# YannisLamp/crypto-recommendation

Measured on AMD Instinct MI355X. Metric: point hash+assign ops/sec at d=128, N=10M, K=256; 1/2/4/8 MI355X, higher is better.
Workload: dtype fp32 points; split-f16 MFMA scores (f32 accumulate); tuples, bucket IDs and cluster IDs bit-exact (x87-exact hashing, certified argmin); distances: certified f32, <= 2^-20 relative to the reference's fp64 (north star: 1e-5; the context's default LSHKM_DIST_CERTIFIED mode), LSHKM_DIST_EXACT for the r; 1 GPU; C3 Lloyd K=256 + C2 LSH L=5 k=4 hashing, N=10000000 per GPU, d=128; N_per_gpu=10000000, N_total=10000000, d=128, K=256, L=5, k=4, nb=100000, parallelism=dp1 (row shards)

## Files before the change

### crypto-recommendation_amd/csrc/fused.hip

```cpp
#include "../../include/lshkm.h"
#include "fused_impl.h"
#include "index.h"

namespace lshkm {

namespace {

struct FusedPlan {
    bool hash = false, cos = false;
    int rows = 0;
    int nblk = 0;
    int64_t seg_rows = 0;
    int np_hi = 0;
    int np_refine = 0;
};

int fused_workspace(lshkm_ctx ctx, const FusedShape& sh, FusedWorkspace& w) {
    const FusedLayout l = fused_layout(sh);
    int rc;
    struct { Buf& b; size_t bytes; } const bufs[] = {
        {ctx->ws_c32, l.c16},      {ctx->ws_cconst, l.cconst}, {ctx->ws_ambig, l.list1}, {ctx->ws_counter, l.counter},
        {ctx->ws_seg, l.seg1},     {ctx->ws_hfix, l.fix},      {ctx->ws_seg3, l.seg3},   {ctx->ws_part, l.part},
        {ctx->ws_ambig2, l.list2}, {ctx->ws_seg2, l.seg2},     {ctx->ws_tuples, l.tuples}, {ctx->ws_cf32, l.cf32},
        {ctx->ws_c64p, l.c64p},    {ctx->ws_xn2, l.xn2}};
// ... 6 lines not shown
    w.nbv = (double*)at(ctx->ws_cconst, l.nbv_off);
    if (l.cf32) { w.C32 = (float*)at(ctx->ws_cf32, 0); w.rn32 = (float*)at(ctx->ws_cf32, l.rn32_off); }
    if (l.c64p) w.C64p = ctx->ws_c64p.as<double>();
    w.list1 = ctx->ws_ambig.as<int32_t>(); w.seg1 = ctx->ws_seg.as<int32_t>();
    w.list2 = ctx->ws_ambig2.as<int32_t>(); w.seg2 = ctx->ws_seg2.as<int32_t>();
    if (l.seg3) w.seg3 = ctx->ws_seg3.as<int32_t>();
    w.hfix = (unsigned long long*)at(ctx->ws_hfix, l.hfix_off);
    w.cfix = (unsigned long long*)at(ctx->ws_hfix, l.cfix_off);
    w.hfix2 = (unsigned long long*)at(ctx->ws_hfix, l.hfix2_off);
    if (l.part) w.part = ctx->ws_part.as<float4>();
    w.cnt = ctx->ws_counter.as<unsigned long long>();
    if (l.xn2) w.xn2 = ctx->ws_xn2.as<double>();
    if (l.tuples) w.tuples = ctx->ws_tuples.as<int32_t>();
    return 0;
}

FusedArgs fused_common_args(lshkm_ctx ctx, const AssignRequest& q, const FusedShape& sh, const FusedWorkspace& w) {
    FusedArgs a{};
    a.X = q.X.f64 ? nullptr : q.X.f(); a.X64 = q.X.f64 ? q.X.d() : nullptr;
    a.N = q.N; a.d = q.d;
    a.xvec = sh.rows == 1 ? (a.d % 4 == 0 && ((uintptr_t)a.X & 15) == 0) : (a.d % 2 == 0 && ((uintptr_t)a.X64 & 15) == 0);
    a.Ch = w.Ch; a.Cl = w.Cl; a.cnh = w.cnh; a.cbound = w.cbound; a.Kpad = sh.Kpad();
    a.C64 = w.C64p ? w.C64p : q.C; a.Cd = q.C;
    a.C32 = w.C32; a.rn32 = w.rn32; a.fast_dist = sh.fast ? 1 : 0;
    a.assign = q.assign; a.dist = q.dist;
    a.stats = ctx->stats.as<unsigned long long>();
    a.nb = 1;
    if (q.lsh) {
        const ProjTable& pj = q.lsh->proj;
        a.Vh = pj.vh_d.as<_Float16>(); a.Vl = pj.vl_d.as<_Float16>(); a.PT = pj.PT_d.as<double>();
        a.tv = pj.t_d.as<float>(); a.pnorm = pj.pn_d.as<double>(); a.v1 = pj.v1_d.as<double>();
        a.rv = pj.r_d.as<int32_t>(); a.w = pj.w; a.L = pj.L; a.k = pj.k; a.LK = pj.LK; a.LKpad = pj.LKpad;
        a.nb = q.lsh->nb;
    }
    a.bdiv = make_bucket_div(a.nb);
    if (sh.cosine) { a.nbv = w.nbv; a.xn2 = w.xn2; }
    a.cfix = w.cfix; a.cfix_counts = w.seg3; a.cfix_count = w.cfix ? w.cnt + CNT_CFIX : nullptr;
    a.pass_first = 1; a.pass_last = 1;
    return a;
}

void hash_outputs(FusedArgs& a, const AssignRequest& q, const FusedShape& sh, const FusedWorkspace& w) {
    a.hfix = w.hfix; a.hfix_count = w.hfix ? w.cnt + CNT_HFIX : nullptr;
    if (!q.lsh) return;
    a.phi = q.phi; a.bucket = q.bucket;
    a.tuples = sh.cosine ? nullptr : q.tuples ? q.tuples : w.tuples;
}

template <typename T>
DevList<T> segmented(T* p, unsigned long long* count, int32_t* counts, const AssignRequest& q, const FusedPlan& plan) {
    DevList<T> l;
    l.p = p; l.count = count; l.bound = q.N; l.counts = counts;
    l.seg_rows = plan.seg_rows; l.nseg = plan.nblk;
    return l;
}

int fused_hi_passes(hipStream_t s, const FusedArgs& hi, const FusedPlan& p) {
    const bool gather_on = !test_switch("LSHKM_GATHER", "0");
    int rc;
    if (p.rows != 0) {
        HiForm h;
        h.metric = p.cos; h.rows = p.rows;
        h.fast = !p.cos && hi.fast_dist;
        h.gath = !p.cos && !h.fast && p.rows == 1 && hi.Kpad <= FH_GATH_KMAX && gather_on;
        return launch_fused_hi_pass(s, p.nblk, h, hi);
    }
    if (!p.cos && p.np_hi == 2 && test_switch("LSHKM_HI_TWO_IMAGE", "1")) {
        HiForm h;
        h.hash = p.hash; h.two_image = true;
        return launch_fused_hi_pass(s, p.nblk, h, hi);
    }
    for (int i = 0; i < p.np_hi; i++) {
        const int c0 = i * FH_KMAX;
        FusedArgs a = hi;
        a.Ch = hi.Ch + (size_t)c0 * FU_D; a.cnh = hi.cnh + c0;
        a.Kpad = std::min(FH_KMAX, hi.Kpad - c0);
        a.t0 = c0 / 32; a.pass_first = i == 0; a.pass_last = i == p.np_hi - 1;
        HiForm h;
        h.hash = p.hash && i == 0; h.mp = p.np_hi > 1; h.metric = p.cos;
        if (!p.cos && !h.mp) {
            const bool small = a.Kpad <= FH_GATH_KMAX && gather_on;
            h.fast = small && a.fast_dist;
            h.gath = small && !a.fast_dist;
        } else if (!p.cos) {
            h.fast = !h.hash && a.fast_dist && a.pass_last;
        }
        if ((rc = launch_fused_hi_pass(s, p.nblk, h, a))) return rc;
    }
    return 0;
}

int fused_refine_passes(hipStream_t s, const FusedArgs& rf, const FusedPlan& p) {
    for (int i = 0; i < p.np_refine; i++) {
        const int c0 = i * FP_KMAX;
        FusedArgs r = rf;
        r.Ch = rf.Ch + (size_t)c0 * FU_D; r.Cl = rf.Cl + (size_t)c0 * FU_D; r.cnh = rf.cnh + c0;
        r.Kpad = std::min(FP_KMAX, rf.Kpad - c0);
        r.t0 = c0 / 32; r.pass_first = i == 0; r.pass_last = i == p.np_refine - 1;
        const int rc = launch_fused_refine_pass(s, (unsigned)p.nblk, p.cos, p.np_refine > 1, p.rows, r);
        if (rc) return rc;
    }
    return 0;
}

struct SideFork {
    lshkm_ctx c;
    bool open = false;
    int fork() {
        if (hipEventRecord(c->fork_ev, c->stream) != hipSuccess ||
            hipStreamWaitEvent(c->side_stream, c->fork_ev, 0) != hipSuccess)
            return kstatus("fused_assign (fork)");
        open = true;
        return 0;
    }
    int end_side() {
        if (c->timing) {
            if (hipEventRecord(c->tev[2], c->side_stream) != hipSuccess) return kstatus("fused_assign (timing)");
            c->tev_side = true;
        }
        if (hipEventRecord(c->join_ev, c->side_stream) != hipSuccess) return kstatus("fused_assign (join)");
        return 0;
    }
    int join() {
        if (!open) return 0;
        if (hipStreamWaitEvent(c->stream, c->join_ev, 0) != hipSuccess) return kstatus("fused_assign (join)");
        open = false;
        return 0;
    }
    ~SideFork() { if (open) (void)hipStreamSynchronize(c->side_stream); }
};

#ifdef LSHKM_PHASE_TIMING
struct PhaseReport {
    hipStream_t s;
    unsigned long long* d = nullptr;
    explicit PhaseReport(hipStream_t s_) : s(s_) {
        static unsigned long long* prof_d = nullptr;
        if (!prof_d) (void)hipMalloc(&prof_d, 64);
        (void)hipMemsetAsync(prof_d, 0, 64, s);
        d = prof_d;
    }
    ~PhaseReport() {
        unsigned long long v[6];
        (void)hipMemcpyAsync(v, d, 48, hipMemcpyDeviceToHost, s);
        (void)hipStreamSynchronize(s);
        fprintf(stderr, "PHASES %llu %llu %llu %llu %llu\n", v[0], v[1], v[2], v[3], v[4]);
    }
};
#endif

}

int fused_assign(lshkm_ctx ctx, const AssignRequest& q) {
    hipStream_t s = ctx->stream;
    const bool cosine = q.metric != LSHKM_METRIC_EUCLIDEAN;
    const ProjTable* pj = q.lsh ? &q.lsh->proj : nullptr;
    const FusedRoute route = fused_route(cosine, q.X.f64, q.d, q.K, pj != nullptr, pj ? pj->k : 0, pj ? pj->LK : 0,
                                         test_switch("LSHKM_FUSED_FORM", "chunked"));
    if (route.form == FusedForm::none || (pj && (q.lsh->metric != q.metric || !pj->mfma_ok))) {
        set_error("fused_assign: no fused form runs this shape (fused_route, fused_layout.h)");
        return LSHKM_ERR_ARG;
    }
    FusedShape sh;
    sh.N = q.N; sh.d = q.d; sh.K = q.K; sh.cosine = cosine; sh.rows = route.rows;
    sh.hash = pj != nullptr; sh.LK = pj ? pj->LK : 0;
    sh.fast = !cosine && sh.rows != 2 && !q.force_exact && ctx->dist_mode == LSHKM_DIST_CERTIFIED;
// ... 92 lines not shown
```

### crypto-recommendation_amd/csrc/fused_hi.hip

```cpp
#include "fused_impl.h"

namespace lshkm {

__host__ __device__ constexpr int fh_lds_bytes(int Kpad, bool hash) {
    return 16 + Kpad * FU_RS * 2 + Kpad * 4 + (hash ? 2 * 32 * FU_RS * 2 + FP_HC_BYTES : 0);
}
static_assert(fh_lds_bytes(FH_KMAX, true) <= 160 * 1024, "hi-only LDS image exceeds 160 KiB");
constexpr double FH_A = 130.0 * 0x1p-23;

constexpr int FH_WAVES_MPFAST = 12;
constexpr int FH_FAST_WAVES = 8;
template <bool HASH, bool MP, int MET, bool FAST = false>
__host__ __device__ constexpr int fh_waves() {
    return HASH && MP ? 12 : (MP && FAST ? FH_WAVES_MPFAST : (FAST && !MP ? FH_FAST_WAVES : 8));
}

__device__ inline int cosine_halves_finish(double sh0, double sl0, double ts0, double sh, double sl, double ts,
                                           double xa, double nbv, double& v) {
    const double mb = 2.0 * sqrt(__dmul_rn(xa, nbv)) * (1.0 + 0x1p-40);
    const double tsum = __dadd_rn(ts0, ts);
    if (!(tsum >= 0x1p-790)) return 2;
    IpAcc ip;
    const double t = __dadd_rn(sh0, sh);
    const double bb = __dsub_rn(t, sh0);
// ... 37 lines not shown
    for (int j = 0; j < 4; j++) cb[j] = *reinterpret_cast<const double2*>(crow_h + 2 * j);
#pragma unroll
    for (int s = 0; s < 8; s++) {
        double cv[8];
#pragma unroll
        for (int j = 0; j < 4; j++) { cv[2 * j] = cb[j].x; cv[2 * j + 1] = cb[j].y; }
        if (s + 1 < 8) {
#pragma unroll
            for (int j = 0; j < 4; j++) cb[j] = *reinterpret_cast<const double2*>(crow_h + 16 * (s + 1) + 2 * j);
        }
#pragma unroll
        for (int j = 0; j < 8; j++) {
            const double pj = __dmul_rn((double)xf[8 * s + j], cv[j]);
            const double t = __dadd_rn(sh, pj);
            const double bb = __dsub_rn(t, sh);
            const double e = __dadd_rn(__dsub_rn(sh, __dsub_rn(t, bb)), __dsub_rn(pj, bb));
            sh = t;
            sl = __dadd_rn(sl, e);
            ts = __dadd_rn(ts, fabs(__dadd_rn(t, off)));
        }
        const double other = swap_halves(sh, h);
        if (h == 1) ts = __dadd_rn(ts, 8.0 * fabs(__dsub_rn(other, off)));
        off = other;
    }
    const double sh0 = swap_halves(sh, h), sl0 = swap_halves(sl, h), ts0 = swap_halves(ts, h);
    if (h == 0) return 2;
    return cosine_halves_finish(sh0, sl0, ts0, sh, sl, ts, xa, nbv, v);
}

__device__ inline int cosine_winner_halves_x64(const FusedArgs& a, int64_t rowc, const double* __restrict__ crow_h,
                                               double nbv, int h, double& v) {
    double2 xn[4], xnn[4];
    load_x64_step(a, rowc, 0, h, xn);
    load_x64_step(a, rowc, 1, h, xnn);
    double sh = 0.0, sl = 0.0, ts = 0.0;
    double off = 0.0;
    double2 cb[4];
#pragma unroll
    for (int j = 0; j < 4; j++) cb[j] = *reinterpret_cast<const double2*>(crow_h + 2 * j);
#pragma unroll 1
    for (int s = 0; s < 8; s++) {
        double xv[8], cv[8];
#pragma unroll
        for (int j = 0; j < 4; j++) {
            xv[2 * j] = xn[j].x; xv[2 * j + 1] = xn[j].y;
            cv[2 * j] = cb[j].x; cv[2 * j + 1] = cb[j].y;
            xn[j] = xnn[j];
        }
        if (s + 2 < 8) load_x64_step(a, rowc, s + 2, h, xnn);
        if (s + 1 < 8) {
#pragma unroll
            for (int j = 0; j < 4; j++) cb[j] = *reinterpret_cast<const double2*>(crow_h + 16 * (s + 1) + 2 * j);
        }
#pragma unroll
        for (int j = 0; j < 8; j++) {
            const double pj = __dmul_rn(xv[j], cv[j]);
            const double t = __dadd_rn(sh, pj);
            const double bb = __dsub_rn(t, sh);
            const double e = __dadd_rn(__dsub_rn(sh, __dsub_rn(t, bb)), __dsub_rn(pj, bb));
            sh = t;
            sl = __dadd_rn(sl, e);
            ts = __dadd_rn(ts, fabs(__dadd_rn(t, off)));
        }
        const double other = swap_halves(sh, h);
        if (h == 1) ts = __dadd_rn(ts, 8.0 * fabs(__dsub_rn(other, off)));
        off = other;
    }
    const double sh0 = swap_halves(sh, h), sl0 = swap_halves(sl, h), ts0 = swap_halves(ts, h);
    if (h == 0) return 2;
    return cosine_halves_finish(sh0, sl0, ts0, sh, sl, ts, a.xn2[rowc], nbv, v);
}

constexpr int FH_GATH_STEP = 32 * 16 * 8;
constexpr int FH_GATH_WAVE = 2 * FH_GATH_STEP;
__host__ __device__ constexpr int fh_gath_off(int Kpad, bool hash) { return (fh_lds_bytes(Kpad, hash) + 255) & ~255; }
static_assert(fh_gath_off(FH_GATH_KMAX, true) + 8 * FH_GATH_WAVE <= 160 * 1024, "gather ring exceeds 160 KiB");

__device__ inline void glds16(const void* gsrc, uint32_t lds_dst) {
    unsigned keep;
    asm volatile("s_mov_b32 %0, m0\n\ts_mov_b32 m0, %2\n\ts_nop 0\n\tglobal_load_lds_dwordx4 %1, off\n\ts_mov_b32 m0, %0"
                 : "=&s"(keep) : "v"(gsrc), "s"(lds_dst) : "memory");
}

template <bool HASH, bool MP = false, int MET = 0, int NIMG = 1, bool GATH = false, int ROWS = 0, bool FAST = false>
__global__ __launch_bounds__((64 * fh_waves<HASH, MP, MET, FAST>()), 1) void fused_hi_kernel(FusedArgs a) {
    constexpr int FH_WAVES = fh_waves<HASH, MP, MET, FAST>();
    constexpr int FH_THREADS = 64 * FH_WAVES;
    static_assert(NIMG == 1 || (!MP && MET == 0), "two-image form: euclidean, single launch");
    static_assert(!GATH || (!MP && MET == 0 && NIMG == 1 && FH_WAVES == 8), "gather ring: euclidean single pass");
    static_assert(ROWS == 0 || (!HASH && !MP && NIMG == 1), "general rows: Lloyd without hashing, one pass");
    static_assert(!(GATH && ROWS == 2), "fp64 rows re-read x in the chain: register loads of the winner rows");
    static_assert(!FAST || (MET == 0 && ROWS != 2 && NIMG == 1 && !GATH), "fast distance: euclidean, fp32 rows");
    extern __shared__ __attribute__((aligned(16))) char smem[];
    const int Kpad = a.Kpad;
    const bool fastd = FAST || a.fast_dist != 0;
    const int KI = NIMG == 2 ? FH_KMAX : Kpad;
    int* lcount = reinterpret_cast<int*>(smem);
    _Float16* lch = reinterpret_cast<_Float16*>(smem + 16);
    float* lcn = reinterpret_cast<float*>(lch + KI * FU_RS);
    _Float16* lvh = reinterpret_cast<_Float16*>(lcn + KI);
    _Float16* lvl = lvh + 32 * FU_RS;
    float* lpn0 = reinterpret_cast<float*>(lvl + 32 * FU_RS);
    float* lv10 = lpn0 + 32;
    float* lt0 = lv10 + 32;
    int32_t* lr0 = reinterpret_cast<int32_t*>(lt0 + 32);

    auto load_image = [&](int img) {
        const int r0 = img * KI, nr = NIMG == 2 && img == 1 ? Kpad - FH_KMAX : KI;
        constexpr int FH_CU = 8;
        for (int e0 = 0; e0 < nr * 16; e0 += FH_THREADS * FH_CU) {
            float4 v[FH_CU];
#pragma unroll
            for (int u = 0; u < FH_CU; u++) {
                const int e = e0 + u * FH_THREADS + (int)threadIdx.x < nr * 16 ? e0 + u * FH_THREADS + (int)threadIdx.x : 0;
                v[u] = *reinterpret_cast<const float4*>(a.Ch + (size_t)(r0 + (e >> 4)) * FU_D + (e & 15) * 8);
            }
#pragma unroll
            for (int u = 0; u < FH_CU; u++) {
                const int e = e0 + u * FH_THREADS + (int)threadIdx.x < nr * 16 ? e0 + u * FH_THREADS + (int)threadIdx.x : 0;
                *reinterpret_cast<float4*>(lch + (e >> 4) * FU_RS + (e & 15) * 8) = v[u];
            }
        }
        for (int e = threadIdx.x; e < nr; e += FH_THREADS) lcn[e] = a.cnh[r0 + e];
    };
    load_image(0);
    if (threadIdx.x < 3) lcount[threadIdx.x] = 0;
    int32_t* ambig_seg = a.ambig + (int64_t)blockIdx.x * a.seg_rows;
    unsigned long long* hfix_seg = a.hfix + (int64_t)blockIdx.x * a.seg_rows;
    unsigned long long* cfix_seg = a.cfix ? a.cfix + (int64_t)blockIdx.x * a.seg_rows : nullptr;
    if (HASH) {
        hash_stage_images<FH_THREADS>(a.Vh, a.Vl, lvh, lvl);
        if (threadIdx.x < 32) {
            const int f = threadIdx.x;
            const bool on = f < a.LK;
            float P = 0.f, Q = 0.f;
            if (on) hash_window<MET == 0>(a.pnorm[f], a.v1[f], MET == 0 ? a.tv[f] : 0.f, a.w, P, Q);
            lpn0[f] = P;
            lv10[f] = Q;
            lt0[f] = on && MET == 0 ? a.tv[f] : 0.f;
            lr0[f] = on && MET == 0 ? a.rv[f] : 0;
        }
    }
    __syncthreads();

    const int lane = threadIdx.x & 63, wave = threadIdx.x >> 6;
    const int col = lane & 31, h = lane >> 5;
    const float cmaxf = a.cbound[3], crf = a.cbound[4], chf = a.cbound[5], cnf = a.cbound[6];
    const bool c_ok = __float_as_uint(a.cbound[2]) == 0u;
    const _Float16* my_h = lch + col * FU_RS + 8 * h;
    const int ntile32 = Kpad >> 5;
    const int64_t ntiles = (a.N + 31) >> 5;
    const double Ec = (0x1p-24 + FH_A) * (double)cnf + 0x1p-41 * (double)cmaxf * (double)cmaxf + 0x1p-18 * (double)cnf;

    const int64_t tstride = (int64_t)gridDim.x * FH_WAVES, tfirst = (int64_t)blockIdx.x * FH_WAVES;
    const int64_t nround = NIMG == 2 && ntiles > tfirst ? (ntiles - tfirst + tstride - 1) / tstride : 0;
    int64_t rd = 0;
    auto load_row = [&](int64_t tl, float (&dst)[64]) {
        const int64_t rr = tl * 32 + col, rc = rr < a.N ? rr : a.N - 1;
        if constexpr (ROWS != 0) load_row_gen<ROWS>(a, rc, h, dst);
        else load_row_b(a.X + rc * FU_D + 8 * h, dst);
    };
    PT_DECL
    for (int64_t tile = tfirst + wave; NIMG == 2 ? rd < nround : tile < ntiles; tile += tstride, rd++) {
        const int64_t row = tile * 32 + col;
        const bool valid = row < a.N;
        float xf[64];
        load_row(tile, xf);
        half8 bh[8];
        float2v n2a = {0.f, 0.f}, n2b = {0.f, 0.f}, r2 = {0.f, 0.f};
        double xn2, nx, nxr, nxh;
        bool x_ok;
        auto finish_norms = [&]() {
            float xn2f = (n2a.x + n2a.y) + (n2b.x + n2b.y);
            float xr2f = r2.x + r2.y;
            xn2f += __shfl_xor(xn2f, 32);
            xr2f += __shfl_xor(xr2f, 32);
            xn2 = (double)xn2f * (1.0 + 0x1p-16);
            nx = sqrt(xn2);
            nxr = sqrt((double)xr2f * (1.0 + 0x1p-16)) + 0x1p-100;
            if (ROWS == 2) nxr += 0x1p-24 * nx * (1.0 + 0x1p-20);
            nxh = nx + nxr;
            x_ok = xn2f <= FU_RANGE * FU_RANGE;
        };
        const bool hash_here = HASH;
        if (!hash_here) {
#pragma unroll
            for (int s = 0; s < 8; s++) {
                half8 unused;
                split_norm_step<false>(xf + 8 * s, bh[s], unused, n2a, n2b, r2);
            }
            finish_norms();
        }

        if (hash_here) {
            uint32_t fmask = 0;
            float acc_hi[16];
            {
                const _Float16* vh_row = lvh + col * FU_RS + 8 * h;
                const _Float16* vl_row = lvl + col * FU_RS + 8 * h;
                floatx16 tot;
#pragma unroll
                for (int s = 0; s < 8; s++) {
                    half8 bl;
                    split_norm_step<true>(xf + 8 * s, bh[s], bl, n2a, n2b, r2);
                    const floatx16 acc = hash_tile_step(s, vh_row, vl_row, bh[s], bl);
                    if (s == 0) {
                        tot = acc;
                    } else {
#pragma unroll
                        for (int r = 0; r < 16; r += 2) {
                            const float2v t2 = {tot[r], tot[r + 1]}, a2 = {acc[r], acc[r + 1]};
                            const float2v u2 = t2 + a2;
                            tot[r] = u2.x;
                            tot[r + 1] = u2.y;
                        }
                    }
                }
#pragma unroll
                for (int r = 0; r < 16; r++) acc_hi[r] = tot[r];
            }
            finish_norms();
            const float iw = MET == 1 ? 1.f : 1.0f / a.w;
            const float nxf = (float)nx * (1.f + 0x1p-20f);
            int hc = 0;
            asm volatile("" : "+v"(hc));
            const float* lt = lt0 + hc;
            const float* lP = lpn0 + hc;
            const float* lQ = lv10 + hc;
            const int32_t* lr = lr0 + hc;
            if (!x_ok && valid) fmask = (a.LK >= 32 ? 0xFFFFFFFFu : (1u << a.LK) - 1u);
#pragma unroll
            for (int g = 0; g < 4; g++) {
                const int l = 2 * g + h;
                if (l >= a.L || !valid) continue;
                const int64_t o = row * a.L + l;
                if constexpr (MET == 1) {
                    int gv = 0;
#pragma unroll
                    for (int q = 0; q < 4; q++) {
                        const int f = 4 * l + q;
                        int bit;
                        if (!certify_sign_f32(acc_hi[4 * g + q], nxf, lP[f], lQ[f], bit)) fmask |= 1u << f;
                        gv = (gv << 1) | bit;
                    }
                    if (a.phi) a.phi[o] = gv;
                    if (a.bucket) a.bucket[o] = gv;
                    continue;
                }
                int32_t hv[4];
#pragma unroll
                for (int q = 0; q < 4; q++) {
                    const int f = 4 * l + q;
                    if (!certify_floor_f32(acc_hi[4 * g + q], lt[f], iw, nxf, lP[f], lQ[f], hv[q])) fmask |= 1u << f;
                }
                if (a.tuples) *reinterpret_cast<int4*>(a.tuples + o * 4) = make_int4(hv[0], hv[1], hv[2], hv[3]);
                uint32_t hn = 0;
#pragma unroll
                for (int q = 0; q < 4; q++) hn += phi_term_small(hv[q], lr[4 * l + q]);
                const uint32_t ph = phi_final(hn);
                if (a.phi) a.phi[o] = (int32_t)ph;
                if (a.bucket) a.bucket[o] = bucket_fast(ph, a.bdiv);
            }
            fmask |= __shfl_xor(fmask, 32);
            const unsigned long long fb = __ballot(fmask != 0u && h == 1);
            if (fb) {
                const int leader = __builtin_ctzll(fb);
                int base = 0;
                if (lane == leader) base = atomicAdd(lcount + 1, __popcll(fb));
                base = __shfl(base, leader);
                if (fmask != 0u && h == 1)
                    hfix_seg[base + __popcll(fb & ((1ull << lane) - 1ull))] = ((unsigned long long)row << 32) | fmask;
            }
        }

        PT_MARK(0)
        const double E = (nxh * (double)crf + nxr * (double)cmaxf + FH_A * nxh * (double)chf + 0x1p-41 * xn2 +
                          0x1p-18 * nx * (double)cmaxf + (MET == 1 ? 0x1p-43 * nx : 0.0) + Ec) * (1.0 + 0x1p-20) +
                         1e-30;
        float m1 = -__builtin_inff(), m2 = -__builtin_inff();
        int t1 = 0;
        if (MP && !HASH && !a.pass_first) {
            const float4 st = a.part[tile * 64 + lane];
            m1 = st.x; m2 = st.y; t1 = __float_as_int(st.z);
        }
        const int tg0 = MP ? a.t0 : 0;
        __builtin_amdgcn_s_setprio(MFMA_PRIO);
        const int ntile_run = ntile32;
        auto run_tiles = [&](int ntl, int tgo) {
#pragma unroll 1
            for (int t = 0; t < ntl; t++) {
                const float m1_prev = m1;
                floatx16 acc;
                const float* cn_t = lcn + t * 32 + 4 * h;
#pragma unroll
                for (int g = 0; g < 4; g++) {
                    const float4 cn = *reinterpret_cast<const float4*>(cn_t + 8 * g);
                    acc[4 * g] = cn.x; acc[4 * g + 1] = cn.y; acc[4 * g + 2] = cn.z; acc[4 * g + 3] = cn.w;
                }
                const _Float16* arow = my_h + t * 32 * FU_RS;
#pragma unroll
                for (int s = 0; s < 8; s++) {
                    const half8 ah = *reinterpret_cast<const half8*>(arow + 16 * s);
                    acc = __builtin_amdgcn_mfma_f32_32x32x16_f16(ah, bh[s], acc, 0, 0, 0);
                }
                float sv[16];
#pragma unroll
                for (int r = 0; r < 16; r++) sv[r] = acc[r];
                tile_epilogue(sv, m1, m2);
                t1 = m1 != m1_prev ? t + tgo : t1;
            }
        };
        if (NIMG == 1) {
            run_tiles(ntile_run, tg0);
        } else {
            const int i0 = (int)(rd & 1);
            const int nA = FH_KMAX / 32, nB = (Kpad - FH_KMAX) / 32;
            run_tiles(i0 == 0 ? nA : nB, i0 * nA);
            __syncthreads();
            load_image(1 - i0);
            __syncthreads();
            run_tiles(i0 == 0 ? nB : nA, (1 - i0) * nA);
        }
        __builtin_amdgcn_s_setprio(0);
        PT_MARK(1)
        if (MP && (HASH || !a.pass_last)) {
            a.part[tile * 64 + lane] = make_float4(m1, m2, __int_as_float(t1), 0.f);
            continue;
        }
        const uint32_t l1 = __float_as_uint(m1) & 0xFu;
        const int i1 = t1 * 32 + 8 * (int)(l1 >> 2) + 4 * h + (int)(l1 & 3u);
        const float om1 = __shfl_xor(m1, 32), om2 = __shfl_xor(m2, 32);
        const int oi1 = __shfl_xor(i1, 32);
        const float M2 = fmaxf(fmaxf(m2, om2), fminf(m1, om1));
        const int I1 = (om1 > m1 || (om1 == m1 && oi1 < i1)) ? oi1 : i1;
        const float M1 = fmaxf(m1, om1);
        const double* crow = a.C64 + (size_t)I1 * FU_D + 8 * h;
        const char* gsrc[4];
        uint32_t gbase = 0;
        const bool g32 = GATH && a.C32 != nullptr && (__float_as_uint(a.cbound[7]) & 1u) == 0u;
        const int gstep = g32 ? 64 : 128;
        if (GATH && !fastd) {
            gbase = (uint32_t)__builtin_amdgcn_readfirstlane(
                (int)((uint32_t)(uintptr_t)(smem + fh_gath_off(Kpad, HASH)) + (uint32_t)wave * FH_GATH_WAVE));
            if (g32) {
#pragma unroll
                for (int u = 0; u < 2; u++) {
                    const int p = 16 * u + (lane >> 2);
                    const int Ip = __shfl(I1, p);
                    gsrc[u] = reinterpret_cast<const char*>(a.C32 + (size_t)Ip * FU_D + 4 * ((lane & 3) ^ ((p >> 2) & 3)));
                }
                gsrc[2] = gsrc[3] = gsrc[0];
#pragma unroll
                for (int s0 = 0; s0 < 2; s0++)
#pragma unroll
                    for (int u = 0; u < 2; u++) glds16(gsrc[u] + gstep * s0, gbase + s0 * FH_GATH_STEP + u * 1024);
            } else {
#pragma unroll
                for (int u = 0; u < 4; u++) {
                    const int p = 8 * u + (lane >> 3);
                    const int Ip = __shfl(I1, p);
                    gsrc[u] = reinterpret_cast<const char*>(a.C64 + (size_t)Ip * FU_D + 2 * ((lane & 7) ^ ((p >> 1) & 7)));
                }
#pragma unroll
                for (int s0 = 0; s0 < 2; s0++)
#pragma unroll
                    for (int u = 0; u < 4; u++) glds16(gsrc[u] + gstep * s0, gbase + s0 * FH_GATH_STEP + u * 1024);
            }
        }
        double2 gnext[4];
        float4 gnext32[2];
        auto gread = [&](int st) {
            const char* ring = smem + fh_gath_off(Kpad, HASH) + wave * FH_GATH_WAVE + (st & 1) * FH_GATH_STEP;
            if (g32) {
#pragma unroll
                for (int j = 0; j < 2; j++)
                    gnext32[j] = *reinterpret_cast<const float4*>(ring + (col >> 4) * 1024 + (col & 15) * 64 +
                                                                  16 * ((2 * h + j) ^ ((col >> 2) & 3)));
            } else {
#pragma unroll
                for (int j = 0; j < 4; j++)
                    gnext[j] = *reinterpret_cast<const double2*>(ring + col * 128 + 16 * ((4 * h + j) ^ ((col >> 1) & 7)));
            }
        };
        auto wait_step = [&]() {
            if (g32) __builtin_amdgcn_s_waitcnt(0x0F72);
            else __builtin_amdgcn_s_waitcnt(0x0F74);
        };
        auto ring_advance = [&](int s) {
            if (s + 2 < 8) {
                __builtin_amdgcn_s_waitcnt(0xC07F);
                asm volatile("" ::: "memory");
                if (g32) {
#pragma unroll
                    for (int u = 0; u < 2; u++) glds16(gsrc[u] + gstep * (s + 2), gbase + (s & 1) * FH_GATH_STEP + u * 1024);
                } else {
#pragma unroll
                    for (int u = 0; u < 4; u++) glds16(gsrc[u] + gstep * (s + 2), gbase + (s & 1) * FH_GATH_STEP + u * 1024);
                }
            }
            if (s + 1 < 8) {
                if (s + 2 < 8) wait_step();
                else __builtin_amdgcn_s_waitcnt(0x0F70);
                asm volatile("" ::: "memory");
                gread(s + 1);
            }
        };
        constexpr int XD = 4;
        double2 xring[XD][4];
        const int64_t rowc = row < a.N ? row : a.N - 1;
        if constexpr (ROWS == 2 && MET == 0) {
#pragma unroll
            for (int st = 0; st < XD; st++) load_x64_step(a, rowc, st, h, xring[st]);
        }
        double2 cbuf[4];
        if (MET == 0 && !GATH && !fastd) {
#pragma unroll
            for (int j = 0; j < 4; j++) cbuf[j] = *reinterpret_cast<const double2*>(crow + 2 * j);
        }
        const bool cert = x_ok && c_ok && ((double)M2 < (double)M1 - 2.0 * E);

        bool dok = true;
        double fdist = 0.0;
        if constexpr (MET == 0) {
            if (fastd) {
                const float* c32 = a.C32 + (size_t)I1 * FU_D + 8 * h;
                float2v q[4] = {};
#pragma unroll
                for (int s = 0; s < 8; s++) {
                    const float4 c0 = *reinterpret_cast<const float4*>(c32 + 16 * s);
                    const float4 c1 = *reinterpret_cast<const float4*>(c32 + 16 * s + 4);
                    const float2v cv[4] = {{c0.x, c0.y}, {c0.z, c0.w}, {c1.x, c1.y}, {c1.z, c1.w}};
#pragma unroll
                    for (int j = 0; j < 4; j++) {
                        const float2v xv = {xf[8 * s + 2 * j], xf[8 * s + 2 * j + 1]};
                        const float2v dv = xv - cv[j];
                        q[j] = __builtin_elementwise_fma(dv, dv, q[j]);
                    }
                }
                float t = ((q[0].x + q[0].y) + (q[1].x + q[1].y)) + ((q[2].x + q[2].y) + (q[3].x + q[3].y));
                t = t + swap_halves_f(t, h);
                const double S = (double)t, R = (double)a.rn32[I1];
                const double B = 14.2 * 0x1p-24 * S + 2.02 * R * sqrt(S) + 2.02 * R * R + 0x1p-100;
                dok = B <= 0x1p-19 * S;
                fdist = sqrt(S);
            }
        }
        const bool amb = valid && !(cert && dok);
        const unsigned long long amask = __ballot(amb && h == 1);
        if (amb && h == 1) {
            int base = 0;
            const int leader = __builtin_ctzll(amask);
            if (lane == leader) base = atomicAdd(lcount, __popcll(amask));
            base = __shfl(base, leader);
            ambig_seg[base + __popcll(amask & ((1ull << lane) - 1ull))] = (int32_t)row;
        }
        if constexpr (MET == 1) {
            bool fix = false;
            if (valid && cert) {
                double v = 0.0;
                int st;
                if constexpr (ROWS == 2) st = cosine_winner_halves_x64(a, row, a.C64 + (size_t)I1 * FU_D + 8 * h, a.nbv[I1], h, v);
                else st = cosine_winner_halves(xf, a.C64 + (size_t)I1 * FU_D + 8 * h, a.nbv[I1], h, v);
                if (h == 1) {
                    a.assign[row] = I1;
                    if (st == 0) a.dist[row] = v;
                    else fix = true;
                }
            }
            const unsigned long long fb = __ballot(fix);
            if (fb) {
                const int leader = __builtin_ctzll(fb);
                int base = 0;
                if (lane == leader) base = atomicAdd(lcount + 2, __popcll(fb));
                base = __shfl(base, leader);
                if (fix) cfix_seg[base + __popcll(fb & ((1ull << lane) - 1ull))] = (unsigned long long)row;
            }
        } else if (fastd) {
            if (h == 1 && valid && cert && dok) {
                a.assign[row] = I1;
                a.dist[row] = fdist;
            }
        } else {
            __builtin_amdgcn_s_setprio(CHAIN_PRIO);
            double acc = 0.0;
            PwAcc pw;
            double* pwl = nullptr;
            if constexpr (ROWS == 2) {
                if (a.pw_lds) pwl = reinterpret_cast<double*>(smem + a.pw_lds) + wave * 512;
            }
            if constexpr (GATH) {
                wait_step();
                asm volatile("" ::: "memory");
                gread(0);
            }
#pragma unroll
            for (int s = 0; s < 8; s++) {
                double sq[8];
                double2 cur[4];
                if constexpr (GATH) {
                    if (g32) {
#pragma unroll
                        for (int j = 0; j < 2; j++) {
                            cur[2 * j] = make_double2((double)gnext32[j].x, (double)gnext32[j].y);
                            cur[2 * j + 1] = make_double2((double)gnext32[j].z, (double)gnext32[j].w);
                        }
                    } else {
#pragma unroll
                        for (int j = 0; j < 4; j++) cur[j] = gnext[j];
                    }
                    ring_advance(s);
                } else {
#pragma unroll
                    for (int j = 0; j < 4; j++) cur[j] = cbuf[j];
                    if (s + 1 < 8) {
#pragma unroll
                        for (int j = 0; j < 4; j++) cbuf[j] = *reinterpret_cast<const double2*>(crow + 16 * (s + 1) + 2 * j);
                    }
                }
                double2 xcur[4];
                if constexpr (ROWS == 2) {
#pragma unroll
                    for (int j = 0; j < 4; j++) xcur[j] = xring[s % XD][j];
                    if (s + XD < 8) load_x64_step(a, rowc, s + XD, h, xring[s % XD]);
                } else {
#pragma unroll
                    for (int j = 0; j < 4; j++) xcur[j] = make_double2((double)xf[8 * s + 2 * j], (double)xf[8 * s + 2 * j + 1]);
                }
                double dv[8];
#pragma unroll
                for (int j = 0; j < 4; j++) {
                    const double2 cc = cur[j];
                    dv[2 * j] = __dsub_rn(xcur[j].x, cc.x);
                    dv[2 * j + 1] = __dsub_rn(xcur[j].y, cc.y);
                }
                if (ROWS == 2 && pwl) {
                    gp_sq_wave<8>(dv, sq, pwl);
                } else {
#pragma unroll
                    for (int j = 0; j < 8; j++) {
                        sq[j] = __dmul_rn(dv[j], dv[j]);
                        pw.add<ROWS == 2>(dv[j]);
                    }
                }
                if (h == 0) {
#pragma unroll
                    for (int j = 0; j < 8; j++) acc = __dadd_rn(acc, sq[j]);
                }
                acc = take_from_lower(acc);
                if (h == 1) {
#pragma unroll
                    for (int j = 0; j < 8; j++) acc = __dadd_rn(acc, sq[j]);
                }
                acc = take_from_upper(acc);
            }
            const bool pw_hard = pwl == nullptr && (pw.hard() || (ROWS != 2 && (__float_as_uint(a.cbound[7]) & 2u) != 0u));
            const int pw_other = __shfl_xor((int)pw_hard, 32);
            const bool hard = pw_hard || pw_other != 0;
            if (h == 1 && valid && cert) {
                a.assign[row] = I1;
                if (!hard) a.dist[row] = sqrt(acc);
            }
            const unsigned long long pb = __ballot(h == 1 && valid && cert && hard);
            if (pb) {
                const int leader = __builtin_ctzll(pb);
                int base = 0;
                if (lane == leader) base = atomicAdd(lcount + 2, __popcll(pb));
                base = __shfl(base, leader);
                if (h == 1 && valid && cert && hard) cfix_seg[base + __popcll(pb & ((1ull << lane) - 1ull))] = (unsigned long long)row;
            }
            __builtin_amdgcn_s_setprio(0);
        }
        PT_MARK(2)
    }
    PT_FLUSH
    __syncthreads();
    if (threadIdx.x < 2 && (!MP || (threadIdx.x == 0 ? (!HASH && a.pass_last != 0) : (HASH && a.pass_first)))) {
        const int c = lcount[threadIdx.x];
        a.seg_counts[SEG_SLOTS * blockIdx.x + threadIdx.x] = c;
        if (c) atomicAdd(threadIdx.x == 0 ? a.ambig_count : a.hfix_count, (unsigned long long)c);
    }
    if ((MET == 1 || !fastd) && threadIdx.x == 2 && (!MP || (!HASH && a.pass_last))) {
        const int c = lcount[2];
        a.cfix_counts[SEG_SLOTS * blockIdx.x + SEG_FIX] = c;
        if (c) atomicAdd(a.cfix_count, (unsigned long long)c);
    }
}

template <bool HASH, bool MP, int MET, int NIMG, bool GATH, int ROWS, bool FAST>
static void hi_launch(hipStream_t s, unsigned nblk, size_t lds, const FusedArgs& a) {
    hipLaunchKernelGGL((fused_hi_kernel<HASH, MP, MET, NIMG, GATH, ROWS, FAST>), dim3(nblk),
                       dim3(64 * fh_waves<HASH, MP, MET, FAST>()), lds, s, a);
}

int launch_fused_hi_pass(hipStream_t s, unsigned nblk, const HiForm& f, FusedArgs a) {
    size_t lds = (size_t)fh_lds_bytes(f.two_image ? FH_KMAX : a.Kpad, f.hash);
    a.pw_lds = 0;
    if (f.gath) {
        if (a.Kpad > FH_GATH_KMAX) {
            set_error("launch_fused_hi_pass: the gather ring needs K <= 256");
            return -1;
        }
        lds = (size_t)fh_gath_off(a.Kpad, f.hash) + 8 * FH_GATH_WAVE;
    } else if (f.rows == 2 && f.metric == 0) {
        constexpr int PW_BYTES = fh_waves<false, false, 0>() * 512 * 8;
        const size_t off = (lds + 255) & ~(size_t)255;
        if (off + PW_BYTES <= 160 * 1024) {
            a.pw_lds = (int)off;
            lds = off + PW_BYTES;
        }
    }
    const int nimg = f.two_image ? 2 : 1;
#define HI_CASE(H, MP, MET, NIMG, GATH, ROWS, FAST)                                                         \
    if (f.hash == (bool)H && f.mp == (bool)MP && f.metric == MET && nimg == NIMG && f.gath == (bool)GATH && \
        f.rows == ROWS && f.fast == (bool)FAST) {                                                           \
        hi_launch<H, MP, MET, NIMG, GATH, ROWS, FAST>(s, nblk, lds, a);                                     \
        return 0;                                                                                           \
    }
    HI_CASE(1, 0, 0, 1, 0, 0, 1)
    HI_CASE(0, 0, 0, 1, 0, 0, 1)
    HI_CASE(1, 0, 0, 1, 1, 0, 0)
    HI_CASE(0, 0, 0, 1, 1, 0, 0)
    HI_CASE(1, 0, 0, 1, 0, 0, 0)
    HI_CASE(0, 0, 0, 1, 0, 0, 0)
    HI_CASE(1, 1, 0, 1, 0, 0, 0)
    HI_CASE(0, 1, 0, 1, 0, 0, 1)
    HI_CASE(0, 1, 0, 1, 0, 0, 0)
    HI_CASE(1, 0, 0, 2, 0, 0, 0)
    HI_CASE(0, 0, 0, 2, 0, 0, 0)
    HI_CASE(1, 0, 1, 1, 0, 0, 0)
    HI_CASE(0, 0, 1, 1, 0, 0, 0)
    HI_CASE(1, 1, 1, 1, 0, 0, 0)
    HI_CASE(0, 1, 1, 1, 0, 0, 0)
    HI_CASE(0, 0, 0, 1, 0, 1, 1)
    HI_CASE(0, 0, 0, 1, 1, 1, 0)
    HI_CASE(0, 0, 0, 1, 0, 1, 0)
    HI_CASE(0, 0, 1, 1, 0, 1, 0)
    HI_CASE(0, 0, 0, 1, 0, 2, 0)
    HI_CASE(0, 0, 1, 1, 0, 2, 0)
#undef HI_CASE
    set_error("launch_fused_hi_pass: no kernel was built for this form");
    return -1;
}

}
```

### crypto-recommendation_amd/csrc/fused_impl.h

```cpp
#pragma once
#include <algorithm>
#include <cstdlib>
#include <cstring>
#include <cstdio>
#include <type_traits>

#include "common.h"
#include "kernels.h"
#include "hash_exact.h"
#include "exact.h"
#include "hash_tile.h"
#include "fused_args.h"

namespace lshkm {

static_assert(FU_D == FUSED_DIMS, "fused_layout.h states the kernels' dimension");
constexpr int FP_THREADS = 64 * FP_WAVES;
constexpr int FH_GATH_KMAX = 256;
constexpr int FP_HC_BYTES = 32 * (4 + 4 + 4 + 4);
constexpr int MFMA_PRIO = 1;
constexpr int CHAIN_PRIO = 2;

struct FusedWorkspace {
    int64_t list_cap = 0;
    _Float16 *Ch = nullptr, *Cl = nullptr;
    float *cbound = nullptr, *cnh = nullptr;
    double* nbv = nullptr;
    float *C32 = nullptr, *rn32 = nullptr;
    double* C64p = nullptr;
    int32_t *list1 = nullptr, *seg1 = nullptr;
    int32_t *list2 = nullptr, *seg2 = nullptr;
    int32_t* seg3 = nullptr;
    unsigned long long *hfix = nullptr, *cfix = nullptr, *hfix2 = nullptr;
    float4* part = nullptr;
    unsigned long long* cnt = nullptr;
    double* xn2 = nullptr;
    int32_t* tuples = nullptr;
};

int launch_fused_prep(hipStream_t s, const double* C, int K, int d, int metric, const FusedWorkspace& w);
int launch_row_sumsq(hipStream_t s, const double* X, int64_t N, int d, double* out);
int launch_fused_chunked(hipStream_t s, bool hash, const FusedArgs& a);
struct HiForm {
    bool hash = false;
    bool mp = false;
    int metric = 0;
    bool two_image = false;
    bool gath = false;
    int rows = 0;
    bool fast = false;
};
int launch_fused_hi_pass(hipStream_t s, unsigned nblk, const HiForm& f, FusedArgs a);
int launch_fused_refine_pass(hipStream_t s, unsigned nblk, int metric, bool mp, int rows, const FusedArgs& a);
void launch_hash_fixup(hipStream_t s, const RecList& l, bool cosine, FusedArgs a);
int launch_cos_fix_seg(hipStream_t s, const AssignJob& q, int nlists, const RecList* lists, const double* xn2,
                       const double* nbv);

#ifdef LSHKM_PHASE_TIMING
#define PT_DECL unsigned long long pt_acc[6] = {0, 0, 0, 0, 0, 0}; unsigned long long pt_t = __builtin_amdgcn_s_memtime();
#define PT_MARK(i) { const unsigned long long t_ = __builtin_amdgcn_s_memtime(); pt_acc[i] += t_ - pt_t; pt_t = t_; }
#define PT_FLUSH if (lane == 0) for (int i_ = 0; i_ < 6; i_++) atomicAdd(a.prof + i_, pt_acc[i_]);
#elif defined(LSHKM_ISA_MARK)
#define PT_DECL
#define PT_MARK(i) asm volatile(";PTMARK " #i);
#define PT_FLUSH
#else
#define PT_DECL
#define PT_MARK(i)
#define PT_FLUSH
#endif

__device__ inline double swap_halves(double v, int h) {
    const uint64_t b = (uint64_t)__double_as_longlong(v);
    const auto lo = __builtin_amdgcn_permlane32_swap((uint32_t)b, (uint32_t)b, false, false);
    const auto hi = __builtin_amdgcn_permlane32_swap((uint32_t)(b >> 32), (uint32_t)(b >> 32), false, false);
    const uint32_t l = h ? lo[0] : lo[1], u = h ? hi[0] : hi[1];
    return __longlong_as_double((long long)(((uint64_t)u << 32) | l));
}

__device__ inline float swap_halves_f(float v, int h) {
    const auto r = __builtin_amdgcn_permlane32_swap(__float_as_uint(v), __float_as_uint(v), false, false);
    return __uint_as_float(h ? r[0] : r[1]);
}

__device__ inline double take_from_lower(double v) {
    const uint64_t b = (uint64_t)__double_as_longlong(v);
    const uint32_t l = __builtin_amdgcn_permlane32_swap((uint32_t)b, (uint32_t)b, false, false)[0];
    const uint32_t u = __builtin_amdgcn_permlane32_swap((uint32_t)(b >> 32), (uint32_t)(b >> 32), false, false)[0];
    return __longlong_as_double((long long)(((uint64_t)u << 32) | l));
}
__device__ inline double take_from_upper(double v) {
    const uint64_t b = (uint64_t)__double_as_longlong(v);
    const uint32_t l = __builtin_amdgcn_permlane32_swap((uint32_t)b, (uint32_t)b, false, false)[1];
    const uint32_t u = __builtin_amdgcn_permlane32_swap((uint32_t)(b >> 32), (uint32_t)(b >> 32), false, false)[1];
    return __longlong_as_double((long long)(((uint64_t)u << 32) | l));
}

__device__ inline void tile_mfma(const _Float16* ah_row, const _Float16* al_row, const half8 (&bh)[8],
                                 const half8 (&bl)[8], floatx16& acc_hi, floatx16& acc_lo) {
#pragma unroll
    for (int r = 0; r < 16; r++) { acc_hi[r] = 0.f; acc_lo[r] = 0.f; }
#pragma unroll
    for (int s = 0; s < 8; s++) {
        const half8 ah = *reinterpret_cast<const half8*>(ah_row + 16 * s);
        const half8 al = *reinterpret_cast<const half8*>(al_row + 16 * s);
        acc_hi = __builtin_amdgcn_mfma_f32_32x32x16_f16(ah, bh[s], acc_hi, 0, 0, 0);
        acc_lo = __builtin_amdgcn_mfma_f32_32x32x16_f16(ah, bl[s], acc_lo, 0, 0, 0);
        acc_lo = __builtin_amdgcn_mfma_f32_32x32x16_f16(al, bh[s], acc_lo, 0, 0, 0);
    }
}

template <int ROWS>
__device__ inline void load_row_gen(const FusedArgs& a, int64_t rowc, int h, float (&dst)[64]) {
    const int64_t ro = rowc * (int64_t)a.d;
#pragma unroll
    for (int s = 0; s < 8; s++) {
        const int j0 = 16 * s + 8 * h;
        if (a.xvec && j0 + 8 <= a.d) {
            if constexpr (ROWS == 1) {
                const float4 p0 = *reinterpret_cast<const float4*>(a.X + ro + j0);
                const float4 p1 = *reinterpret_cast<const float4*>(a.X + ro + j0 + 4);
                dst[8 * s + 0] = p0.x; dst[8 * s + 1] = p0.y; dst[8 * s + 2] = p0.z; dst[8 * s + 3] = p0.w;
                dst[8 * s + 4] = p1.x; dst[8 * s + 5] = p1.y; dst[8 * s + 6] = p1.z; dst[8 * s + 7] = p1.w;
            } else {
#pragma unroll
                for (int j = 0; j < 4; j++) {
                    const double2 q = *reinterpret_cast<const double2*>(a.X64 + ro + j0 + 2 * j);
                    dst[8 * s + 2 * j] = (float)q.x;
                    dst[8 * s + 2 * j + 1] = (float)q.y;
                }
            }
        } else {
#pragma unroll
// ... 41 lines not shown
```

Measured before the change: 4.903 billion point hash+assign ops/s.

## Prefetch next point tile via LDS DMA and registers in fast hi kernel

```diff
diff --git a/crypto-recommendation_amd/csrc/fused.hip b/crypto-recommendation_amd/csrc/fused.hip
--- a/crypto-recommendation_amd/csrc/fused.hip
+++ b/crypto-recommendation_amd/csrc/fused.hip
@@ -112,6 +112,7 @@
             const bool small = a.Kpad <= FH_GATH_KMAX && gather_on;
             h.fast = small && a.fast_dist;
             h.gath = small && !a.fast_dist;
+            h.rowpf = h.fast && !test_switch("LSHKM_ROW_PREFETCH", "0");
         } else if (!p.cos) {
             h.fast = !h.hash && a.fast_dist && a.pass_last;
         }
diff --git a/crypto-recommendation_amd/csrc/fused_hi.hip b/crypto-recommendation_amd/csrc/fused_hi.hip
--- a/crypto-recommendation_amd/csrc/fused_hi.hip
+++ b/crypto-recommendation_amd/csrc/fused_hi.hip
@@ -143,7 +143,25 @@
                  : "=&s"(keep) : "v"(gsrc), "s"(lds_dst) : "memory");
 }
 
-template <bool HASH, bool MP = false, int MET = 0, int NIMG = 1, bool GATH = false, int ROWS = 0, bool FAST = false>
+#ifndef LSHKM_ROWPF
+#define LSHKM_ROWPF 3
+#endif
+constexpr int FH_ROWPF = LSHKM_ROWPF;
+constexpr int FH_ROWPF_KMAX = 256;
+constexpr int FH_ROWPF_WAVE = 32 * 64 * 4;
+__host__ __device__ constexpr int fh_rowpf_off(int Kpad, bool hash) { return (fh_lds_bytes(Kpad, hash) + 255) & ~255; }
+static_assert(fh_rowpf_off(FH_ROWPF_KMAX, true) + FH_FAST_WAVES * FH_ROWPF_WAVE <= 160 * 1024,
+              "row prefetch buffers exceed 160 KiB");
+static_assert(FH_ROWPF_KMAX <= FH_GATH_KMAX, "the FAST single-pass form runs where the gather ring would (fused.hip)");
+
+__device__ inline void glds16s(const void* sbase, uint32_t voff, uint32_t lds_base, int lds_off) {
+    unsigned keep;
+    asm volatile("s_mov_b32 %0, m0\n\ts_add_u32 m0, %3, %4\n\ts_nop 0\n\tglobal_load_lds_dwordx4 %1, %2\n\ts_mov_b32 m0, %0"
+                 : "=&s"(keep) : "v"(voff), "s"(sbase), "s"(lds_base), "n"(lds_off) : "memory", "scc");
+}
+
+template <bool HASH, bool MP = false, int MET = 0, int NIMG = 1, bool GATH = false, int ROWS = 0, bool FAST = false,
+          int PF = 0>
 __global__ __launch_bounds__((64 * fh_waves<HASH, MP, MET, FAST>()), 1) void fused_hi_kernel(FusedArgs a) {
     constexpr int FH_WAVES = fh_waves<HASH, MP, MET, FAST>();
     constexpr int FH_THREADS = 64 * FH_WAVES;
@@ -152,6 +170,8 @@
     static_assert(ROWS == 0 || (!HASH && !MP && NIMG == 1), "general rows: Lloyd without hashing, one pass");
     static_assert(!(GATH && ROWS == 2), "fp64 rows re-read x in the chain: register loads of the winner rows");
     static_assert(!FAST || (MET == 0 && ROWS != 2 && NIMG == 1 && !GATH), "fast distance: euclidean, fp32 rows");
+    static_assert(PF == 0 || (FAST && !MP && ROWS == 0 && FH_WAVES == FH_FAST_WAVES), "row prefetch: the FAST single-pass form");
+    constexpr bool PFR = (PF & 1) != 0, PFL = (PF & 2) != 0;
     extern __shared__ __attribute__((aligned(16))) char smem[];
     const int Kpad = a.Kpad;
     const bool fastd = FAST || a.fast_dist != 0;
@@ -204,7 +224,8 @@
     }
     __syncthreads();
 
-    const int lane = threadIdx.x & 63, wave = threadIdx.x >> 6;
+    const int lane = threadIdx.x & 63;
+    const int wave = PF != 0 ? __builtin_amdgcn_readfirstlane((int)(threadIdx.x >> 6)) : (int)(threadIdx.x >> 6);
     const int col = lane & 31, h = lane >> 5;
     const float cmaxf = a.cbound[3], crf = a.cbound[4], chf = a.cbound[5], cnf = a.cbound[6];
     const bool c_ok = __float_as_uint(a.cbound[2]) == 0u;
@@ -221,12 +242,94 @@
         if constexpr (ROWS != 0) load_row_gen<ROWS>(a, rc, h, dst);
         else load_row_b(a.X + rc * FU_D + 8 * h, dst);
     };
+    auto load_half = [&](int64_t tl, int hf, float* dst) {
+        const int64_t rr = tl * 32 + col, rc = rr < a.N ? rr : a.N - 1;
+        const float* xr = a.X + rc * FU_D + 64 * hf + 8 * h;
+#pragma unroll
+        for (int s = 0; s < 4; s++) {
+            const float4 p0 = *reinterpret_cast<const float4*>(xr + 16 * s);
+            const float4 p1 = *reinterpret_cast<const float4*>(xr + 16 * s + 4);
+            dst[8 * s + 0] = p0.x; dst[8 * s + 1] = p0.y; dst[8 * s + 2] = p0.z; dst[8 * s + 3] = p0.w;
+            dst[8 * s + 4] = p1.x; dst[8 * s + 5] = p1.y; dst[8 * s + 6] = p1.z; dst[8 * s + 7] = p1.w;
+        }
+    };
+    uint32_t pfbase = 0;
+    if constexpr (PFL)
+        pfbase = (uint32_t)__builtin_amdgcn_readfirstlane(
+            (int)((uint32_t)(uintptr_t)(smem + fh_rowpf_off(Kpad, HASH)) + (uint32_t)wave * FH_ROWPF_WAVE));
+    auto pf_dma = [&](int64_t tl) {
+        const int64_t tls = ((int64_t)__builtin_amdgcn_readfirstlane((int)(tl >> 32)) << 32) |
+                            (uint32_t)__builtin_amdgcn_readfirstlane((int)tl);
+        const int64_t left = a.N - 1 - tls * 32;
+        const int pmax = left < 31 ? (int)left : 31;
+        const float* xt = a.X + tls * 32 * FU_D;
+        if (pmax == 31) {
+            const uint32_t w0 = (uint32_t)((lane >> 4) * (FU_D * 4) + 16 * ((lane & 15) ^ (lane >> 4)));
+#pragma unroll
+            for (int u = 0; u < 8; u++) glds16s(xt + u * 4 * FU_D, w0 ^ (uint32_t)(64 * (u & 3)), pfbase, u * 1024);
+        } else {
+#pragma unroll
+            for (int u = 0; u < 8; u++) {
+                const int p = 4 * u + (lane >> 4), pc = p < pmax ? p : pmax;
+                glds16s(xt, (uint32_t)(pc * (FU_D * 4) + 16 * ((lane & 15) ^ (p & 15))), pfbase, u * 1024);
+            }
+        }
+    };
+    float xn[32];
+    auto pf_next = [&](int64_t tl) {
+        if constexpr (PF != 0) {
+            if (tl + tstride < ntiles) {
+                if constexpr (PFL) {
+                    __builtin_amdgcn_s_waitcnt(0xC07F);
+                    asm volatile("" ::: "memory");
+                    pf_dma(tl + tstride);
+                }
+                if constexpr (PFR) load_half(tl + tstride, 1, xn);
+            } else if constexpr (PFR) {
+#pragma unroll
+                for (int j = 0; j < 32; j++) xn[j] = 0.f;
+            }
+        }
+    };
+    if constexpr (PF != 0) {
+        if (tfirst + wave < ntiles) {
+            if constexpr (PFL) pf_dma(tfirst + wave);
+            if constexpr (PFR) load_half(tfirst + wave, 1, xn);
+            if constexpr (PFL) {
+                __builtin_amdgcn_s_waitcnt(0x0F70);
+                asm volatile("" ::: "memory");
+            }
+        }
+    }
     PT_DECL
     for (int64_t tile = tfirst + wave; NIMG == 2 ? rd < nround : tile < ntiles; tile += tstride, rd++) {
         const int64_t row = tile * 32 + col;
         const bool valid = row < a.N;
         float xf[64];
-        load_row(tile, xf);
+        if constexpr (PF == 0) {
+            load_row(tile, xf);
+        } else {
+            if constexpr (PFL) {
+                if constexpr (!PFR) {
+                    load_half(tile, 1, xf + 32);
+                    asm volatile("" ::: "memory");
+                }
+                __builtin_amdgcn_s_waitcnt(PFR ? 0x4F70 : 0x0F78);
+                asm volatile("" ::: "memory");
+                const char* pb = smem + fh_rowpf_off(Kpad, HASH) + wave * FH_ROWPF_WAVE + col * 256;
+#pragma unroll
+                for (int c = 0; c < 8; c++) {
+                    const float4 v = *reinterpret_cast<const float4*>(pb + 16 * ((4 * (c >> 1) + 2 * h + (c & 1)) ^ (col & 15)));
+                    xf[4 * c] = v.x; xf[4 * c + 1] = v.y; xf[4 * c + 2] = v.z; xf[4 * c + 3] = v.w;
+                }
+            } else {
+                load_half(tile, 0, xf);
+            }
+            if constexpr (PFR) {
+#pragma unroll
+                for (int j = 0; j < 32; j++) xf[32 + j] = xn[j];
+            }
+        }
         half8 bh[8];
         float2v n2a = {0.f, 0.f}, n2b = {0.f, 0.f}, r2 = {0.f, 0.f};
         double xn2, nx, nxr, nxh;
@@ -250,6 +353,7 @@
                 half8 unused;
                 split_norm_step<false>(xf + 8 * s, bh[s], unused, n2a, n2b, r2);
             }
+            pf_next(tile);
             finish_norms();
         }
 
@@ -334,6 +438,7 @@
             }
         }
 
+        if (HASH) pf_next(tile);
         PT_MARK(0)
         const double E = (nxh * (double)crf + nxr * (double)cmaxf + FH_A * nxh * (double)chf + 0x1p-41 * xn2 +
                           0x1p-18 * nx * (double)cmaxf + (MET == 1 ? 0x1p-43 * nx : 0.0) + Ec) * (1.0 + 0x1p-20) +
@@ -486,10 +591,24 @@
             if (fastd) {
                 const float* c32 = a.C32 + (size_t)I1 * FU_D + 8 * h;
                 float2v q[4] = {};
+                float4 cc[16];
+                if constexpr (PF != 0) {
+#pragma unroll
+                    for (int s = 0; s < 8; s++) {
+                        cc[2 * s] = *reinterpret_cast<const float4*>(c32 + 16 * s);
+                        cc[2 * s + 1] = *reinterpret_cast<const float4*>(c32 + 16 * s + 4);
+                    }
+                    __builtin_amdgcn_sched_barrier(0);
+                }
 #pragma unroll
                 for (int s = 0; s < 8; s++) {
-                    const float4 c0 = *reinterpret_cast<const float4*>(c32 + 16 * s);
-                    const float4 c1 = *reinterpret_cast<const float4*>(c32 + 16 * s + 4);
+                    float4 c0, c1;
+                    if constexpr (PF != 0) {
+                        c0 = cc[2 * s]; c1 = cc[2 * s + 1];
+                    } else {
+                        c0 = *reinterpret_cast<const float4*>(c32 + 16 * s);
+                        c1 = *reinterpret_cast<const float4*>(c32 + 16 * s + 4);
+                    }
                     const float2v cv[4] = {{c0.x, c0.y}, {c0.z, c0.w}, {c1.x, c1.y}, {c1.z, c1.w}};
 #pragma unroll
                     for (int j = 0; j < 4; j++) {
@@ -647,9 +766,9 @@
     }
 }
 
-template <bool HASH, bool MP, int MET, int NIMG, bool GATH, int ROWS, bool FAST>
+template <bool HASH, bool MP, int MET, int NIMG, bool GATH, int ROWS, bool FAST, int PF>
 static void hi_launch(hipStream_t s, unsigned nblk, size_t lds, const FusedArgs& a) {
-    hipLaunchKernelGGL((fused_hi_kernel<HASH, MP, MET, NIMG, GATH, ROWS, FAST>), dim3(nblk),
+    hipLaunchKernelGGL((fused_hi_kernel<HASH, MP, MET, NIMG, GATH, ROWS, FAST, PF>), dim3(nblk),
                        dim3(64 * fh_waves<HASH, MP, MET, FAST>()), lds, s, a);
 }
 
@@ -670,13 +789,22 @@
             lds = off + PW_BYTES;
         }
     }
+    const int pf = f.rowpf ? FH_ROWPF : 0;
+    if (pf != 0 && !(f.fast && !f.mp && f.rows == 0 && !f.gath && a.Kpad <= FH_ROWPF_KMAX)) {
+        set_error("launch_fused_hi_pass: the row prefetch needs the fast single-pass form at K <= 256");
+        return -1;
+    }
+    if (pf & 2) lds = (size_t)fh_rowpf_off(a.Kpad, f.hash) + FH_FAST_WAVES * FH_ROWPF_WAVE;
     const int nimg = f.two_image ? 2 : 1;
-#define HI_CASE(H, MP, MET, NIMG, GATH, ROWS, FAST)                                                         \
+#define HI_CASE_PF(H, MP, MET, NIMG, GATH, ROWS, FAST, PF)                                                  \
     if (f.hash == (bool)H && f.mp == (bool)MP && f.metric == MET && nimg == NIMG && f.gath == (bool)GATH && \
-        f.rows == ROWS && f.fast == (bool)FAST) {                                                           \
-        hi_launch<H, MP, MET, NIMG, GATH, ROWS, FAST>(s, nblk, lds, a);                                     \
+        f.rows == ROWS && f.fast == (bool)FAST && pf == PF) {                                               \
+        hi_launch<H, MP, MET, NIMG, GATH, ROWS, FAST, PF>(s, nblk, lds, a);                                 \
         return 0;                                                                                           \
     }
+#define HI_CASE(H, MP, MET, NIMG, GATH, ROWS, FAST) HI_CASE_PF(H, MP, MET, NIMG, GATH, ROWS, FAST, 0)
+    HI_CASE_PF(1, 0, 0, 1, 0, 0, 1, FH_ROWPF)
+    HI_CASE_PF(0, 0, 0, 1, 0, 0, 1, FH_ROWPF)
     HI_CASE(1, 0, 0, 1, 0, 0, 1)
     HI_CASE(0, 0, 0, 1, 0, 0, 1)
     HI_CASE(1, 0, 0, 1, 1, 0, 0)
@@ -699,6 +827,7 @@
     HI_CASE(0, 0, 0, 1, 0, 2, 0)
     HI_CASE(0, 0, 1, 1, 0, 2, 0)
 #undef HI_CASE
+#undef HI_CASE_PF
     set_error("launch_fused_hi_pass: no kernel was built for this form");
     return -1;
 }
diff --git a/crypto-recommendation_amd/csrc/fused_impl.h b/crypto-recommendation_amd/csrc/fused_impl.h
--- a/crypto-recommendation_amd/csrc/fused_impl.h
+++ b/crypto-recommendation_amd/csrc/fused_impl.h
@@ -49,6 +49,7 @@
     bool gath = false;
     int rows = 0;
     bool fast = false;
+    bool rowpf = false;
 };
 int launch_fused_hi_pass(hipStream_t s, unsigned nblk, const HiForm& f, FusedArgs a);
 int launch_fused_refine_pass(hipStream_t s, unsigned nblk, int metric, bool mp, int rows, const FusedArgs& a);
```

Result: faster. 5.064 billion point hash+assign ops/s, median of 6 (+3.3%).
